# mborhi/CoMA-UNet

Measured on AMD Instinct MI355X. Metric: volumes/sec (train fwd+bwd) at 128^3 bf16, higher is better.
Workload: dtype bf16; 1 GPU; CoMA-UNet train step (fwd + RoiMSE/RnC loss + bwd + all-reduce + AdamW), 128^3 volumes, batch 2/GPU, 6-dim covariates (BASELINE configs[3]); global_batch=2, parallelism=dp1, launch=hipGraph replay of the whole step

## Files before the change

### coma_unet_amd/csrc/conv_mfma.hip

```cpp
#include "common.h"
#include "conv_tiles.h"
#include <type_traits>

template <typename T> struct elem;
template <> struct elem<bf16_t> { static constexpr int EPB = 8; };
template <> struct elem<float> { static constexpr int EPB = 4; };

__device__ __forceinline__ f32x16_t mma_piece(const uint4& a, const uint4& b, f32x16_t acc, bf16_t) {
  return __builtin_amdgcn_mfma_f32_32x32x16_bf16(*reinterpret_cast<const bf16x8_t*>(&a), *reinterpret_cast<const bf16x8_t*>(&b), acc, 0, 0, 0);
}
__device__ __forceinline__ f32x16_t mma_piece(const uint4& a, const uint4& b, f32x16_t acc, float) {
  acc = __builtin_amdgcn_mfma_f32_32x32x2f32(__uint_as_float(a.x), __uint_as_float(b.x), acc, 0, 0, 0);
  acc = __builtin_amdgcn_mfma_f32_32x32x2f32(__uint_as_float(a.y), __uint_as_float(b.y), acc, 0, 0, 0);
  acc = __builtin_amdgcn_mfma_f32_32x32x2f32(__uint_as_float(a.z), __uint_as_float(b.z), acc, 0, 0, 0);
  acc = __builtin_amdgcn_mfma_f32_32x32x2f32(__uint_as_float(a.w), __uint_as_float(b.w), acc, 0, 0, 0);
  return acc;
}

struct GatherP {
  const void* x; int ldx; long sbx; int Di, Hi, Wi, C;
  void* y; int ldy; long sby; int Do, Ho, Wo, N;
  const void* w; long wsb;
  const float* bias; int bsb;
  int k, stride, flip;
// ... 1072 lines not shown
        }
        const char* Wc = Wl + ((ph >> 1) & 1) * WB + w_frag;
        constexpr int NXR = LX == 5 ? 4 : 5;
        uint4 wg[2][3], xr[2][NXR];
        auto rdg = [&](int g, int bf) {
          const int kz = g / 3, kx = g % 3;
          const int toff = (kz * HY * HX + kx) * P;
#pragma unroll
          for (int r = 0; r < NXR; ++r) xr[bf][r] = *reinterpret_cast<const uint4*>(Hl + a_base + toff + r * HX * P);
#pragma unroll
          for (int ky = 0; ky < 3; ++ky) wg[bf][ky] = *reinterpret_cast<const uint4*>(Wc + (kz * 9 + ky * 3 + kx) * 1024);
        };
        rdg(0, 0);
#pragma unroll
        for (int g = 0; g < 9; ++g) {
          if (g + 1 < 9) rdg(g + 1, (g + 1) & 1);
#pragma unroll
          for (int ky = 0; ky < 3; ++ky)
#pragma unroll
            for (int i = 0; i < 2; ++i) acc[i] = mma_piece(wg[g & 1][ky], xr[g & 1][RY * i + ky], acc[i], bf16_t());
          __builtin_amdgcn_sched_group_barrier(0x008, 1, 0); __builtin_amdgcn_sched_group_barrier(0x100, 2, 0);
          __builtin_amdgcn_sched_group_barrier(0x008, 1, 0); __builtin_amdgcn_sched_group_barrier(0x100, 2, 0);
          __builtin_amdgcn_sched_group_barrier(0x008, 1, 0); __builtin_amdgcn_sched_group_barrier(0x100, 1, 0);
          __builtin_amdgcn_sched_group_barrier(0x008, 1, 0); __builtin_amdgcn_sched_group_barrier(0x100, 1, 0);
          __builtin_amdgcn_sched_group_barrier(0x008, 1, 0); __builtin_amdgcn_sched_group_barrier(0x100, 1, 0);
          __builtin_amdgcn_sched_group_barrier(0x008, 1, 0);
          __builtin_amdgcn_sched_barrier(0);
        }
      }
  };
  auto other_phase = [&](auto odd_c, int ph) __attribute__((always_inline)) {
      constexpr int odd = decltype(odd_c)::value;
#ifdef COMA_DUO_NO_STAGE
      if (cC.valid && cC.cc == nch - 1) {
#pragma unroll
        for (int i = 0; i < 2; ++i) asm volatile("" :: "v"(acc[i]));
      }
      cC = cB; advance(cB);
      return;
#endif
      store_halo(odd_c);
      const int ws = (ph >> 1) + 1;
      if (w_needed(ws)) store_w(ws);
      __builtin_amdgcn_s_waitcnt(0x0F70);
      if constexpr (odd == 0) {
#ifdef COMA_DUO_NO_EPI
      if (cC.valid && cC.cc == nch - 1) {
#pragma unroll
        for (int i = 0; i < 2; ++i) asm volatile("" :: "v"(acc[i]));
      }
#else
      if (cC.valid && cC.cc == nch - 1) {
        const int x0 = cC.tix * TX, y0 = cC.tiy * TY, z0 = cC.tiz * TZ;
        float4 bq[4];
#pragma unroll
        for (int g4 = 0; g4 < 4; ++g4) bq[g4] = *reinterpret_cast<const float4*>(bias_l + 8 * g4 + 4 * fh);
#pragma unroll
        for (int i = 0; i < 2; ++i) {
          const int j = wq * 2 + i;
          const int gz = z0 + (j >> 2), gy = y0 + (j & 3) * RY + (fr >> LX), gx = x0 + (fr & (TX - 1));
          const bool valid = gz < p.D && gy < p.H && gx < p.W;
          unsigned pk[4][2];
#pragma unroll
          for (int g4 = 0; g4 < 4; ++g4) {
            bf16_t o[4];
            const float bv[4] = {bq[g4].x, bq[g4].y, bq[g4].z, bq[g4].w};
#pragma unroll
            for (int q = 0; q < 4; ++q) {
              o[q] = static_cast<bf16_t>(acc[i][g4 * 4 + q] + bv[q]);
              if constexpr (STATS) {
                const float r = valid ? static_cast<float>(o[q]) : 0.f;
                st_s[g4][q] += r; st_q[g4][q] = fmaf(r, r, st_q[g4][q]);
              }
            }
            const uint2 u = *reinterpret_cast<const uint2*>(o);
            pk[g4][0] = u.x; pk[g4][1] = u.y;
          }
          bf16_t* vox = yb + ((long)(gz * p.H + gy) * p.W + gx) * p.ldy + n0 + 8 * fh;
#pragma unroll
          for (int gp = 0; gp < 2; ++gp) {
            const auto r0 = __builtin_amdgcn_permlane32_swap(pk[2 * gp][0], pk[2 * gp + 1][0], false, false);
            const auto r1 = __builtin_amdgcn_permlane32_swap(pk[2 * gp][1], pk[2 * gp + 1][1], false, false);
            if (valid) *reinterpret_cast<uint4*>(vox + 16 * gp) = make_uint4(r0[0], r1[0], r0[1], r1[1]);
          }
          __builtin_amdgcn_sched_barrier(0);
        }
      }
#endif
      }
      cC = cB; advance(cB);
      if constexpr (odd == 1) { load_halo(cA); advance2(cA); }
      if (w_needed(ws + 1)) load_w(ws + 1, true);
  };
  __builtin_amdgcn_s_waitcnt(0x0F70);
  if (grp == 0) {
#pragma unroll 1
    for (int ph = 0; ph < nphases; ph += 4) {
      matrix_phase(ph); duo_barrier(); other_phase(odd_t{}, ph + 1); duo_barrier();
      matrix_phase(ph + 2); duo_barrier(); other_phase(even_t{}, ph + 3); duo_barrier();
    }
  } else {
#pragma unroll 1
    for (int ph = 0; ph < nphases; ph += 4) {
      other_phase(even_t{}, ph); duo_barrier(); matrix_phase(ph + 1); duo_barrier();
      other_phase(odd_t{}, ph + 2); duo_barrier(); matrix_phase(ph + 3); duo_barrier();
    }
  }

  if constexpr (STATS) {
    if (p.stats) {
      asm volatile("s_waitcnt vmcnt(0)" ::: "memory");
      __syncthreads();
      float* red = reinterpret_cast<float*>(smem);
#pragma unroll
      for (int g4 = 0; g4 < 4; ++g4)
#pragma unroll
        for (int q = 0; q < 4; ++q) {
          float a = st_s[g4][q], c = st_q[g4][q];
#pragma unroll
          for (int o = 16; o > 0; o >>= 1) { a += __shfl_xor(a, o, 64); c += __shfl_xor(c, o, 64); }
          if (fr == 0) { red[(wid * 32 + 8 * g4 + 4 * fh + q) * 2] = a; red[(wid * 32 + 8 * g4 + 4 * fh + q) * 2 + 1] = c; }
        }
      __syncthreads();
      if (tid < 32 && n0 + tid < p.N) {
        double a = 0.0, c = 0.0;
        for (int w = 0; w < 8; ++w) { a += (double)red[(w * 32 + tid) * 2]; c += (double)red[(w * 32 + tid) * 2 + 1]; }
        const int g = p.stats_inst ? b : 0;
        stat_add(p.stats, p.stats_inst ? p.stats_inst : 1, p.N, g, n0 + tid, a, c);
      }
    }
  }
}

typedef __attribute__((ext_vector_type(4))) float f32x4_t;

struct Thin16P {
  const bf16_t* x; int ldx; long sbx; int D, H, W, C;
  bf16_t* y; int ldy; long sby; int N;
  const bf16_t* w; long wsb;
  const float* bias; int bsb;
  int flip;
  unsigned xbytes;
  int ntx, nty, ntz, ids_total, ids_per_block;
  int st8;
  double2* stats; int stats_inst;
};

template <int CP, int NB>
__global__ __launch_bounds__(256, 2) void conv_thin16_k(Thin16P p) {
  constexpr int TX = 32, TY = 4, TZ = 2, HX = TX + 2, HY = TY + 2, HZ = TZ + 2, HV = HX * HY * HZ;
  constexpr int TPM = 32 / CP, NM = (27 + TPM - 1) / TPM;
  constexpr int PCH = CP / 8;
  constexpr int P = CP * 2;
  constexpr int HP = HV * PCH, HIT = (HP + 255) / 256;
  extern __shared__ __attribute__((aligned(16))) char smem[];
  char* Hl = smem;
  const int tid = threadIdx.x, lane = tid & 63;
  const int wid = __builtin_amdgcn_readfirstlane(tid >> 6);
  const int b = blockIdx.z;
#ifdef COMA_STAMPS
  unsigned long long st_acc[8] = {0, 0, 0, 0, 0, 0, 0, 0};
  const unsigned long long st_begin = stamp_now();
  bool st_first = true;
#endif
  const int lv = lane & 15, lg = lane >> 4;
  const bf16_t* xb = p.x + (long)b * p.sbx;
  const bf16_t* wb = p.w + (long)b * p.wsb;
  bf16_t* yb = p.y + (long)b * p.sby;

  const int tsub = CP == 16 ? lg >> 1 : lg, cofs = CP == 16 ? 8 * (lg & 1) : 0;
  {
    const int total = 27 * p.N * p.C;
    unsigned short* Wl = reinterpret_cast<unsigned short*>(smem);
    const unsigned short* wg = reinterpret_cast<const unsigned short*>(wb);
    if ((total & 7) == 0 && (((uintptr_t)wg) & 15) == 0) {
      for (int i = tid; i < (total >> 3); i += 256) reinterpret_cast<uint4*>(Wl)[i] = reinterpret_cast<const uint4*>(wg)[i];
    } else {
      for (int i = tid; i < total; i += 256) Wl[i] = wg[i];
    }
  }
  __syncthreads();
  bf16x8_t wf[NM][NB];
#pragma unroll
  for (int m = 0; m < NM; ++m) {
    const int tap = m * TPM + tsub;
    const int wt = p.flip ? 26 - tap : tap;
#pragma unroll
    for (int nb = 0; nb < NB; ++nb) {
      const int n = nb * 16 + lv;
      unsigned short e[8];
#pragma unroll
      for (int j = 0; j < 8; ++j) {
        const int c = cofs + j;
        const bool ok = tap < 27 && n < p.N && c < p.C;
        const unsigned short v = reinterpret_cast<const unsigned short*>(smem)[ok ? (wt * p.N + n) * p.C + c : 0];
        e[j] = ok ? v : (unsigned short)0;
      }
      wf[m][nb] = (bf16x8_t){(short)e[0], (short)e[1], (short)e[2], (short)e[3], (short)e[4], (short)e[5], (short)e[6], (short)e[7]};
    }
  }
  const int gz = wid >> 1, gy0 = 2 * (wid & 1);
  int abase[NM];
#pragma unroll
  for (int m = 0; m < NM; ++m) {
    const int tap = m * TPM + tsub < 27 ? m * TPM + tsub : 0;
    const int kx = tap % 3, ky = (tap / 3) % 3, kz = tap / 9;
    abase[m] = (((gz + kz) * HY + gy0 + ky) * HX + lv + kx) * P + cofs * 2;
  }
  const __amdgpu_buffer_rsrc_t rs_x = __builtin_amdgcn_make_buffer_rsrc(const_cast<bf16_t*>(xb), 0, p.xbytes, 0x00020000);
  constexpr unsigned OOB = 0x7fff0000u;
  int h_z[HIT], h_y[HIT], h_x[HIT], h_lds[HIT];
  unsigned h_boff[HIT];
#pragma unroll
  for (int it = 0; it < HIT; ++it) {
    const int piece = tid + 256 * it;
    const int row = piece / PCH, ch = piece % PCH;
    const int hx = row % HX, hy = (row / HX) % HY, hz = row / (HX * HY);
    h_z[it] = piece < HP ? hz : (1 << 20); h_y[it] = hy; h_x[it] = hx;
#ifdef COMA_ABLATE_HALO
    if (hz < 1 || hz > TZ || hy < 1 || hy > TY || hx < 1 || hx > TX) h_z[it] = 1 << 20;
#endif
    h_boff[it] = (unsigned)((((hz * p.H + hy) * p.W + hx) * p.ldx + ch * 8) * 2);
    h_lds[it] = row * P + ch * 16;
  }
  const uint4 hmask = mask8(p.C - 8 * (tid % PCH));
  uint4 hreg[HIT];
  auto issue = [&](int it, int z0, int y0, int x0) __attribute__((always_inline)) {
    const bool ok = (unsigned)(z0 - 1 + h_z[it]) < (unsigned)p.D && (unsigned)(y0 - 1 + h_y[it]) < (unsigned)p.H &&
                    (unsigned)(x0 - 1 + h_x[it]) < (unsigned)p.W;
    const unsigned org_b = (unsigned)((((long)((z0 - 1) * p.H + (y0 - 1)) * p.W + (x0 - 1)) * p.ldx) * 2);
    const auto v = __builtin_amdgcn_raw_buffer_load_b128(rs_x, ok ? org_b + h_boff[it] : OOB, 0, 0);
    hreg[it] = make_uint4(v[0], v[1], v[2], v[3]);
  };
  auto store_halo = [&]() __attribute__((always_inline)) {
#pragma unroll
    for (int it = 0; it < HIT; ++it)
      if (tid + 256 * it < HP) {
        const uint4 m = hmask;
        uint4 v = hreg[it];
        v.x &= m.x; v.y &= m.y; v.z &= m.z; v.w &= m.w;
        *reinterpret_cast<uint4*>(Hl + h_lds[it]) = v;
      }
  };

  const int id_begin = xcd_remap(blockIdx.x, gridDim.x) * p.ids_per_block;
  int id_end = id_begin + p.ids_per_block;
  if (id_end > p.ids_total) id_end = p.ids_total;
  int id = id_begin, tix = 0, tiy = 0, tiz = 0;
  while (id < id_end && !tile_coords(id, p.ntx, p.nty, p.ntz, tix, tiy, tiz)) ++id;
  const bool do_stats = p.stats != nullptr;
  float st_s[NB][4], st_q[NB][4], bv[NB][4];
#pragma unroll
  for (int nb = 0; nb < NB; ++nb)
#pragma unroll
    for (int j = 0; j < 4; ++j) {
      const int n = nb * 16 + 4 * lg + j;
      st_s[nb][j] = 0.f; st_q[nb][j] = 0.f;
      bv[nb][j] = (p.bias && n < p.N) ? p.bias[b * p.bsb + n] : 0.f;
    }
  if (id < id_end) {
#pragma unroll
    for (int it = 0; it < HIT; ++it) issue(it, tiz * TZ, tiy * TY, tix * TX);
  }
  while (id < id_end) {
    const int x0 = tix * TX, y0 = tiy * TY, z0 = tiz * TZ;
    int nid = id + 1, ntix = 0, ntiy = 0, ntiz = 0;
    while (nid < id_end && !tile_coords(nid, p.ntx, p.nty, p.ntz, ntix, ntiy, ntiz)) ++nid;
    const bool has_next = nid < id_end;
    const __amdgpu_buffer_rsrc_t rs_n = __builtin_amdgcn_make_buffer_rsrc(const_cast<bf16_t*>(xb), 0, has_next ? p.xbytes : 0, 0x00020000);
    STAMP(t0);
#ifdef COMA_STAMPS
    if (st_first) { st_acc[0] += t0 - st_begin; st_first = false; }
#endif
    __syncthreads();
    STAMP(t1);
#ifdef COMA_STAMPS
    asm volatile("s_waitcnt vmcnt(0)" ::: "memory");
#endif
    STAMP(t2);
    store_halo();
    __syncthreads();
    STAMP(t3);
    f32x4_t acc[4][NB];
#pragma unroll
    for (int q = 0; q < 4; ++q)
#pragma unroll
      for (int nb = 0; nb < NB; ++nb) acc[q][nb] = (f32x4_t){0.f, 0.f, 0.f, 0.f};
    uint4 fr[3][4];
    auto ldfrag = [&](int m, int q) __attribute__((always_inline)) {
      return *reinterpret_cast<const uint4*>(Hl + abase[m] + ((q >> 1) * HX + (q & 1) * 16) * P);
    };
#pragma unroll
    for (int q = 0; q < 4; ++q) { fr[0][q] = ldfrag(0, q); fr[1][q] = ldfrag(1, q); }
#pragma unroll
    for (int m = 0; m < NM; ++m) {
      if (m + 2 < NM) {
#pragma unroll
        for (int q = 0; q < 4; ++q) fr[(m + 2) % 3][q] = ldfrag(m + 2, q);
      }
      if (m < HIT) {
        const int it = m;
        const bool ok = (unsigned)(ntiz * TZ - 1 + h_z[it]) < (unsigned)p.D && (unsigned)(ntiy * TY - 1 + h_y[it]) < (unsigned)p.H &&
                        (unsigned)(ntix * TX - 1 + h_x[it]) < (unsigned)p.W;
        const unsigned org_b = (unsigned)((((long)((ntiz * TZ - 1) * p.H + (ntiy * TY - 1)) * p.W + (ntix * TX - 1)) * p.ldx) * 2);
        const auto v = __builtin_amdgcn_raw_buffer_load_b128(rs_n, ok ? org_b + h_boff[it] : OOB, 0, 0);
        hreg[it] = make_uint4(v[0], v[1], v[2], v[3]);
      }
      __builtin_amdgcn_sched_barrier(0);
#ifdef COMA_ABLATE_MFMA
      if (m > 0) continue;
#endif
#pragma unroll
      for (int q = 0; q < 4; ++q) {
        const uint4 f = fr[m % 3][q];
#pragma unroll
        for (int nb = 0; nb < NB; ++nb)
          acc[q][nb] = __builtin_amdgcn_mfma_f32_16x16x32_bf16(wf[m][nb], *reinterpret_cast<const bf16x8_t*>(&f), acc[q][nb], 0, 0, 0);
      }
      __builtin_amdgcn_sched_barrier(0);
    }
    static_assert(HIT <= NM, "one staging piece per MFMA step");
    STAMP(t4);
#pragma unroll
    for (int q = 0; q < 4; ++q) {
      const int vz = z0 + gz, vy = y0 + gy0 + (q >> 1), vx = x0 + (q & 1) * 16 + lv;
      const bool valid = vz < p.D && vy < p.H && vx < p.W;
      bf16_t* vox = yb + ((long)(vz * p.H + vy) * p.W + vx) * p.ldy;
#pragma unroll
      for (int nb = 0; nb < NB; ++nb) {
        const int n = nb * 16 + 4 * lg;
        if (n >= p.N) continue;
        bf16_t o[4];
#pragma unroll
        for (int j = 0; j < 4; ++j) {
          o[j] = static_cast<bf16_t>(acc[q][nb][j] + bv[nb][j]);
          if (do_stats) { const float r = valid ? static_cast<float>(o[j]) : 0.f; st_s[nb][j] += r; st_q[nb][j] = fmaf(r, r, st_q[nb][j]); }
        }
#ifdef COMA_ABLATE_STORE
        if (valid && acc[q][nb][0] == 123.456f) {
#else
        if (valid) {
#endif
          if (p.st8 && n + 3 < p.N) *reinterpret_cast<uint2*>(vox + n) = *reinterpret_cast<const uint2*>(o);
          else {
#pragma unroll
            for (int j = 0; j < 4; ++j) if (n + j < p.N) vox[n + j] = o[j];
          }
        }
      }
    }
    id = nid; tix = ntix; tiy = ntiy; tiz = ntiz;
    STAMP(t5);
    STAMP_ADD(1, t0, t1); STAMP_ADD(2, t1, t2); STAMP_ADD(3, t2, t3); STAMP_ADD(4, t3, t4); STAMP_ADD(5, t4, t5);
  }
#ifdef COMA_STAMPS
  {
    const unsigned long long st_end = stamp_now();
    if (lane == 0) {
      for (int k = 0; k < 7; ++k) atomicAdd(&g_stamps[k], st_acc[k]);
      atomicAdd(&g_stamps[7], st_end - st_begin);
      atomicAdd(&g_stamps[8], 1ull);
    }
  }
#endif
  if (p.stats) {
    __syncthreads();
    float* red = reinterpret_cast<float*>(smem);
#pragma unroll
    for (int nb = 0; nb < NB; ++nb)
#pragma unroll
      for (int j = 0; j < 4; ++j) {
        float a = st_s[nb][j], c = st_q[nb][j];
#pragma unroll
        for (int o = 8; o > 0; o >>= 1) { a += __shfl_xor(a, o, 64); c += __shfl_xor(c, o, 64); }
        if (lv == 0) { red[(wid * 32 + nb * 16 + 4 * lg + j) * 2] = a; red[(wid * 32 + nb * 16 + 4 * lg + j) * 2 + 1] = c; }
      }
    __syncthreads();
    if (tid < NB * 16 && tid < p.N) {
      double a = 0.0, c = 0.0;
      for (int w = 0; w < 4; ++w) { a += (double)red[(w * 32 + tid) * 2]; c += (double)red[(w * 32 + tid) * 2 + 1]; }
      const int g = p.stats_inst ? b : 0;
      stat_add(p.stats, p.stats_inst ? p.stats_inst : 1, p.N, g, tid, a, c);
    }
  }
}

struct Thin16FP {
  const float* x; int ldx; long sbx; int D, H, W, C;
  float* y; int ldy; long sby; int N;
  const float* w; long wsb;
  const float* bias; int bsb;
  int flip;
  unsigned xbytes;
  int ntx, nty, ntz, ids_total, ids_per_block;
  int st16;
  double2* stats; int stats_inst;
};

template <int CP, int NB>
__global__ __launch_bounds__(256, 2) void conv_thin16f_k(Thin16FP p) {
  constexpr int TX = 32, TY = 4, TZ = 2, HX = TX + 2, HY = TY + 2, HZ = TZ + 2, HV = HX * HY * HZ;
  constexpr int CQ = CP / 4;
  constexpr int P = CP * 4;
  constexpr int PCH = CP / 4;
  constexpr int HP = HV * PCH, HIT = (HP + 255) / 256;
  constexpr int WROW = NB * 16;
  extern __shared__ __attribute__((aligned(16))) char smem[];
  char* Hl = smem;
  float* Wl = reinterpret_cast<float*>(smem + HV * P);
  const int tid = threadIdx.x, lane = tid & 63;
  const int wid = __builtin_amdgcn_readfirstlane(tid >> 6);
  const int b = blockIdx.z;
  const int lv = lane & 15, lg = lane >> 4;
  const float* xb = p.x + (long)b * p.sbx;
  const float* wb = p.w + (long)b * p.wsb;
  float* yb = p.y + (long)b * p.sby;

  for (int i = tid; i < 27 * WROW * CP; i += 256) {
    const int c = i % CP, n = (i / CP) % WROW, t = i / (CP * WROW);
    const int wt = p.flip ? 26 - t : t;
    const bool ok = n < p.N && c < p.C;
    const float v = wb[ok ? ((long)wt * p.N + n) * p.C + c : 0];
    Wl[i] = ok ? v : 0.f;
  }
  const int gz = wid >> 1, gy0 = 2 * (wid & 1);
  const int xbase = ((gz * HY + gy0) * HX + lv) * P + lg * CQ * 4;
  const int wbase = (lv * CP + lg * CQ) * 4;
  const __amdgpu_buffer_rsrc_t rs_x = __builtin_amdgcn_make_buffer_rsrc(const_cast<float*>(xb), 0, p.xbytes, 0x00020000);
  constexpr unsigned OOB = 0x7fff0000u;
  int h_z[HIT], h_y[HIT], h_x[HIT];
  unsigned h_boff[HIT];
#pragma unroll
  for (int it = 0; it < HIT; ++it) {
    const int piece = tid + 256 * it;
    const int row = piece / PCH, ch = piece % PCH;
    const int hx = row % HX, hy = (row / HX) % HY, hz = row / (HX * HY);
    h_z[it] = piece < HP ? hz : (1 << 20); h_y[it] = hy; h_x[it] = hx;
    h_boff[it] = (unsigned)((((hz * p.H + hy) * p.W + hx) * p.ldx + ch * 4) * 4);
  }
  const int nval = p.C - 4 * (tid % PCH);
  const uint4 hmask = make_uint4(nval > 0 ? ~0u : 0u, nval > 1 ? ~0u : 0u, nval > 2 ? ~0u : 0u, nval > 3 ? ~0u : 0u);
  uint4 hreg[HIT];
  auto store_halo = [&]() __attribute__((always_inline)) {
#pragma unroll
    for (int it = 0; it < HIT; ++it)
      if (tid + 256 * it < HP) {
        uint4 v = hreg[it];
        v.x &= hmask.x; v.y &= hmask.y; v.z &= hmask.z; v.w &= hmask.w;
        *reinterpret_cast<uint4*>(Hl + (tid + 256 * it) * 16) = v;
      }
  };

  const int id_begin = xcd_remap(blockIdx.x, gridDim.x) * p.ids_per_block;
  int id_end = id_begin + p.ids_per_block;
  if (id_end > p.ids_total) id_end = p.ids_total;
  int id = id_begin, tix = 0, tiy = 0, tiz = 0;
  while (id < id_end && !tile_coords(id, p.ntx, p.nty, p.ntz, tix, tiy, tiz)) ++id;
  const bool do_stats = p.stats != nullptr;
  float st_s[NB][4], st_q[NB][4], bv[NB][4];
#pragma unroll
  for (int nb = 0; nb < NB; ++nb)
#pragma unroll
    for (int j = 0; j < 4; ++j) {
      const int n = nb * 16 + 4 * lg + j;
      st_s[nb][j] = 0.f; st_q[nb][j] = 0.f;
      bv[nb][j] = (p.bias && n < p.N) ? p.bias[b * p.bsb + n] : 0.f;
    }
  if (id < id_end) {
#pragma unroll
    for (int it = 0; it < HIT; ++it) {
      const int z0 = tiz * TZ, y0 = tiy * TY, x0 = tix * TX;
      const bool ok = (unsigned)(z0 - 1 + h_z[it]) < (unsigned)p.D && (unsigned)(y0 - 1 + h_y[it]) < (unsigned)p.H &&
                      (unsigned)(x0 - 1 + h_x[it]) < (unsigned)p.W;
      const unsigned org_b = (unsigned)((((long)((z0 - 1) * p.H + (y0 - 1)) * p.W + (x0 - 1)) * p.ldx) * 4);
      const auto v = __builtin_amdgcn_raw_buffer_load_b128(rs_x, ok ? org_b + h_boff[it] : OOB, 0, 0);
      hreg[it] = make_uint4(v[0], v[1], v[2], v[3]);
    }
  }
  while (id < id_end) {
    const int x0 = tix * TX, y0 = tiy * TY, z0 = tiz * TZ;
    int nid = id + 1, ntix = 0, ntiy = 0, ntiz = 0;
    while (nid < id_end && !tile_coords(nid, p.ntx, p.nty, p.ntz, ntix, ntiy, ntiz)) ++nid;
    const bool has_next = nid < id_end;
    const __amdgpu_buffer_rsrc_t rs_n = __builtin_amdgcn_make_buffer_rsrc(const_cast<float*>(xb), 0, has_next ? p.xbytes : 0, 0x00020000);
    __syncthreads();
    store_halo();
    __syncthreads();
    f32x4_t acc[4][NB];
#pragma unroll
    for (int q = 0; q < 4; ++q)
#pragma unroll
      for (int nb = 0; nb < NB; ++nb) acc[q][nb] = (f32x4_t){0.f, 0.f, 0.f, 0.f};
    float xf[2][4][CQ], wfr[2][NB][CQ];
    auto rd = [&](int t, int bf) __attribute__((always_inline)) {
      const int toff = (((t / 9) * HY + (t / 3) % 3) * HX + t % 3) * P;
#pragma unroll
      for (int q = 0; q < 4; ++q) {
        const char* src = Hl + xbase + toff + ((q >> 1) * HX + (q & 1) * 16) * P;
        if constexpr (CQ == 4) { const float4 v = *reinterpret_cast<const float4*>(src); xf[bf][q][0] = v.x; xf[bf][q][1] = v.y; xf[bf][q][2] = v.z; xf[bf][q][3] = v.w; }
        else if constexpr (CQ == 2) { const float2 v = *reinterpret_cast<const float2*>(src); xf[bf][q][0] = v.x; xf[bf][q][1] = v.y; }
        else xf[bf][q][0] = *reinterpret_cast<const float*>(src);
      }
#pragma unroll
      for (int nb = 0; nb < NB; ++nb) {
        const char* src = reinterpret_cast<const char*>(Wl) + wbase + (t * WROW + nb * 16) * CP * 4;
        if constexpr (CQ == 4) { const float4 v = *reinterpret_cast<const float4*>(src); wfr[bf][nb][0] = v.x; wfr[bf][nb][1] = v.y; wfr[bf][nb][2] = v.z; wfr[bf][nb][3] = v.w; }
// ... 622 lines not shown
    (void)hipFuncSetAttribute((const void*)conv_mfma_tconv_k<float, true>, hipFuncAttributeMaxDynamicSharedMemorySize, 160 * 1024);
    attr = true;
  }
  const size_t lds = (size_t)(33 * 5 * 3 + 14 * 32) * 80;
  coma_set_kernel_tag("conv_mfma_tconv_k<%s, %d>", sizeof(T) == 2 ? "__bf16" : "float", q.stats ? 1 : 0);
  const dim3 grid((unsigned)gx, (unsigned)nblk_n, (unsigned)x->B);
  if (q.stats) hipLaunchKernelGGL((conv_mfma_tconv_k<T, true>), grid, dim3(256), lds, s, q);
  else hipLaunchKernelGGL((conv_mfma_tconv_k<T, false>), grid, dim3(256), lds, s, q);
  COMA_LAUNCH_CHECK();
  return 0;
}

bool conv_mfma_supported(const coma_conv_desc* d, const coma_tensor* x, const coma_tensor* y) {
  if (x->dtype != COMA_BF16 || y->dtype != COMA_BF16) return false;
  if ((long)t_vox(x) * x->ld >= (1L << 31) || (long)t_vox(y) * y->ld >= (1L << 31)) return false;
  if (halo_ok(d, x, y)) return true;
  if (pw_ok(d, x, y)) return true;
  if (x->C % 32 || y->C % 32) return false;
  if (x->ld % 8 || y->ld % 8 || x->sb % 8 || y->sb % 8) return false;
  if (x->data && !aligned16(x->data)) return false;
  if ((long)t_vox(x) * x->ld >= (1L << 31) || (long)t_vox(y) * y->ld >= (1L << 31)) return false;
  if (d->form == 1 && d->stride == 2 && d->ksize != 3) return false;
  return true;
}

static bool f32_halo_ok(const coma_conv_desc* d, const coma_tensor* x, const coma_tensor* y) {
  if (x->W < 16 && x->C % 32 == 0 && y->C % 32 == 0) return false;
  return d->ksize == 3 && d->stride == 1 && x->W >= 8 && (long)x->H * x->W >= 32 && x->C % 16 == 0 && y->C >= 16 &&
         x->ld % 4 == 0 && x->sb % 4 == 0 && (!x->data || aligned16(x->data)) && (unsigned long long)t_vox(x) * x->ld * 4 < 0x7fff0000ull;
}
bool conv_f32mfma_supported(const coma_conv_desc* d, const coma_tensor* x, const coma_tensor* y) {
  if (x->dtype != COMA_F32 || y->dtype != COMA_F32) return false;
  if ((long)t_vox(x) * x->ld >= (1L << 31) || (long)t_vox(y) * y->ld >= (1L << 31)) return false;
  if (thin16f_ok(d, x, y)) return true;
  if (f32_halo_ok(d, x, y)) return true;
  if (x->C % 16 || y->C % 32) return false;
  if (x->ld % 4 || y->ld % 4 || x->sb % 4 || y->sb % 4) return false;
  if (x->data && !aligned16(x->data)) return false;
  if (d->form == 1 && d->stride == 2 && d->ksize != 3) return false;
  return true;
}

static int gather_ksplit(long blocks, int nsteps, bool f32) {
  if (f32) {
    if (blocks >= 192 || nsteps < 8) return 1;
    long ks = 256 / blocks;
    if (ks > 8) ks = 8;
    if (ks > nsteps / 4) ks = nsteps / 4;
    return ks < 2 ? 1 : (int)ks;
  }
  if (blocks >= 384 || nsteps < 16) return 1;
  long ks = 512 / blocks;
  if (ks > 8) ks = 8;
  if (ks > nsteps / 4) ks = nsteps / 4;
  return ks < 2 ? 1 : (int)ks;
}

template <int BN, typename T>
static int launch_gather(const GatherP& p0, int mode, int B, hipStream_t s, void* ws, size_t ws_bytes, int ws_zeroed,
                         double2* stats, int stats_inst, int* stats_chunks) {
  GatherP p = p0;
  constexpr int BM = (BN == 128) ? 128 : 256;
  constexpr int LCK = elem<T>::EPB == 8 ? 5 : 4;
  const long Mtot = (long)p.Mz * p.My * p.Mx;
  const size_t lds = (size_t)2 * (BM + BN) * 64 + BM * 4;
  const unsigned gx = (unsigned)((Mtot + BM - 1) / BM), gy = (unsigned)(p.N / BN) * (mode == 1 ? 8 : 1);
  const long Vout = (long)p.Do * p.Ho * p.Wo;
  const int ntaps_max = mode == 1 ? 8 : p.k * p.k * p.k;
  p.ksplit = gather_ksplit((long)gx * gy * B, (mode == 1 ? 1 : ntaps_max) * (p.C >> LCK), LCK == 4);
  p.part = nullptr; p.part_sb = 0;
  if (p.ksplit > 1 && ws && ws_bytes >= sizeof(float) * (size_t)B * Vout * p.N) {
    p.part = (float*)ws; p.part_sb = Vout * p.N;
    if (!ws_zeroed && hipMemsetAsync(ws, 0, sizeof(float) * (size_t)B * Vout * p.N, s) != hipSuccess) { coma_set_error("conv split-K memset failed"); return 2; }
  } else p.ksplit = 1;
  p.stats = nullptr; p.stats_inst = stats_inst;
  if (stats && p.ksplit == 1 && !p.accum) { p.stats = stats; *stats_chunks = 1; }
  dim3 grid(gx, gy * p.ksplit, (unsigned)B);
  coma_set_kernel_tag("conv_mfma_gather_k<%d, %d, %s>", BN, mode, LCK == 4 ? "float" : "__bf16");
  if (mode == 0) hipLaunchKernelGGL((conv_mfma_gather_k<BN, 0, T>), grid, dim3(256), lds, s, p);
  else hipLaunchKernelGGL((conv_mfma_gather_k<BN, 1, T>), grid, dim3(256), lds, s, p);
  COMA_LAUNCH_CHECK();
  if (p.ksplit > 1) {
    long nb = (Vout * p.N + 255) / 256;
    if (nb > 1024) nb = 1024;
    hipLaunchKernelGGL(gather_finalize_k<T>, dim3((unsigned)nb, (unsigned)B), dim3(256), 0, s, (const float*)p.part, p.part_sb, (T*)p.y, p.ldy,
                       p.sby, p.N, Vout, p.bias, p.bsb, p.accum);
    COMA_LAUNCH_CHECK();
  }
  return 0;
}

template <int CK, int LX, int VEC, typename T>
static int launch_halo(const HaloP& p0, int B, hipStream_t s) {
  HaloP p = p0;
  constexpr int TX = 1 << LX, RY = 32 / TX, TY = 4 * RY, TZ = 2;
  constexpr int HV = (TX + 2) * (TY + 2) * (TZ + 2);
  p.ntx = (p.W + TX - 1) / TX; p.nty = (p.H + TY - 1) / TY; p.ntz = (p.D + TZ - 1) / TZ;
  const size_t lds = (size_t)(HV + 9 * 32) * CK * sizeof(T);
  static bool attr = false;
  if (!attr) { (void)hipFuncSetAttribute((const void*)conv_mfma_halo_k<CK, LX, VEC, T>, hipFuncAttributeMaxDynamicSharedMemorySize, 96 * 1024); attr = true; }
  dim3 grid((unsigned)(p.ntx * p.nty * ((p.ntz + 7) / 8) * 8), (unsigned)((p.N + 31) / 32), (unsigned)B);
  coma_set_kernel_tag("conv_mfma_halo_k<%d, %d, %d, %s>", CK, LX, VEC, sizeof(T) == 4 ? "float" : "__bf16");
  hipLaunchKernelGGL((conv_mfma_halo_k<CK, LX, VEC, T>), grid, dim3(256), lds, s, p);
  COMA_LAUNCH_CHECK();
  return 0;
}

static bool aligned16(const void* p);
static size_t duo_frag_bytes(const coma_conv_desc* d, const coma_tensor* x, const coma_tensor* y) {
  static const bool on = getenv("COMA_DUO_C32_ONLY") == nullptr && getenv("COMA_NO_DUO") == nullptr;
  if (!on || x->dtype != COMA_BF16 || d->ksize != 3 || d->stride != 1 || x->W < 16) return 0;
  if (x->C < 64 || x->C % 16 || y->C % 32) return 0;
  return (size_t)(d->per_sample_w ? x->B : 1) * 27 * y->C * x->C * 2;
}

template <typename T>
static int conv_mfma_halo(const coma_conv_desc* d, const coma_tensor* x, const void* wk, const float* bias,
                          const coma_tensor* y, hipStream_t s, double2* stats = nullptr, int stats_inst = 0,
                          int* stats_chunks = nullptr, void* ws = nullptr, size_t ws_bytes = 0) {
  constexpr int EPB = elem<T>::EPB;
  constexpr bool F32 = EPB == 4;
  HaloP p;
  p.x = x->data; p.ldx = (int)x->ld; p.sbx = x->sb; p.D = x->D; p.H = x->H; p.W = x->W; p.C = x->C;
  p.y = y->data; p.ldy = (int)y->ld; p.sby = y->sb; p.N = y->C;
  p.w = wk; p.wsb = d->per_sample_w ? 27L * y->C * x->C : 0;
  p.bias = bias; p.bsb = d->per_sample_w ? y->C : 0;
  p.flip = d->form == 1;
  p.vecx = x->ld % EPB == 0 && x->sb % EPB == 0 && aligned16(x->data);
  p.vecw = x->C % EPB == 0 && aligned16(wk);
  const bool thin = !F32 && x->C <= 16;
  const int lx = x->W >= 32 ? 5 : (x->W >= 16 ? 4 : 3);
  const bool vec = p.vecx && p.vecw && x->C % (4 * EPB) == 0 && (unsigned long long)t_vox(x) * x->ld * sizeof(T) < 0x7fff0000ull;
  if (F32) COMA_CHECK(vec, "conv_mfma(fp32): operands must allow 16-byte channel pieces (C %% 16 == 0, aligned)");
  if constexpr (!F32) {
    static const bool thin16_on = []{ const char* e = getenv("COMA_THIN16"); return !(e && e[0] == '0'); }();
    const unsigned long long xb_ = (unsigned long long)t_vox(x) * x->ld * sizeof(T);
    if (thin16_on && thin && lx == 5 && y->C <= (x->C > 8 ? 16 : 32) && p.vecx && xb_ < 0x7fff0000ull) {
      Thin16P q;
      q.x = (const bf16_t*)p.x; q.ldx = p.ldx; q.sbx = p.sbx; q.D = p.D; q.H = p.H; q.W = p.W; q.C = p.C;
      q.y = (bf16_t*)p.y; q.ldy = p.ldy; q.sby = p.sby; q.N = p.N; q.w = (const bf16_t*)p.w; q.wsb = p.wsb; q.bias = p.bias; q.bsb = p.bsb;
      q.flip = p.flip; q.xbytes = (unsigned)xb_;
      q.st8 = y->ld % 4 == 0 && y->sb % 4 == 0 && (((uintptr_t)y->data) & 7) == 0;
      q.ntx = (q.W + 31) / 32; q.nty = (q.H + 3) / 4; q.ntz = (q.D + 1) / 2;
      q.ids_total = q.ntx * q.nty * ((q.ntz + 7) / 8) * 8;
      int gx = 1024 / x->B;
      if (gx < 1) gx = 1;
      if (gx > q.ids_total) gx = q.ids_total;
      q.ids_per_block = (q.ids_total + gx - 1) / gx;
      gx = (q.ids_total + q.ids_per_block - 1) / q.ids_per_block;
      q.stats = nullptr; q.stats_inst = stats_inst;
      if (stats) { q.stats = stats; *stats_chunks = 1; }
      dim3 grid((unsigned)gx, 1, (unsigned)x->B);
      const bool c16 = q.C > 8, n32 = q.N > 16;
      size_t lds = (size_t)34 * 6 * 4 * (c16 ? 32 : 16);
      if (lds < (size_t)27 * q.N * q.C * 2) lds = (size_t)27 * q.N * q.C * 2;
      coma_set_kernel_tag("conv_thin16_k<%d, %d>", c16 ? 16 : 8, n32 ? 2 : 1);
      if (c16) hipLaunchKernelGGL((conv_thin16_k<16, 1>), grid, dim3(256), lds, s, q);
      else     { if (n32) hipLaunchKernelGGL((conv_thin16_k<8, 2>), grid, dim3(256), lds, s, q);  else hipLaunchKernelGGL((conv_thin16_k<8, 1>), grid, dim3(256), lds, s, q); }
      COMA_LAUNCH_CHECK();
      return 0;
    }
  }
  if ((lx == 5 && (thin || vec)) || (lx == 4 && !F32 && !thin && vec)) {
    Halo2P q;
    q.x = p.x; q.ldx = p.ldx; q.sbx = p.sbx; q.D = p.D; q.H = p.H; q.W = p.W; q.C = p.C;
    q.y = p.y; q.ldy = p.ldy; q.sby = p.sby; q.N = p.N; q.w = p.w; q.wsb = p.wsb; q.bias = p.bias; q.bsb = p.bsb;
    q.flip = p.flip; q.vecx = p.vecx; q.vecw = p.vecw;
    {
      const unsigned long long xb_ = (unsigned long long)t_vox(x) * x->ld * sizeof(T), wb_ = 27ull * y->C * x->C * sizeof(T);
      q.xbytes = (unsigned)(xb_ < 0x7fff0000ull ? xb_ : 0x7fff0000ull);
      q.wbytes = (unsigned)(wb_ < 0x7fff0000ull ? wb_ : 0x7fff0000ull);
    }
    q.stats = nullptr; q.stats_inst = stats_inst;
    q.st8 = y->ld % 4 == 0 && y->sb % 4 == 0 && (((uintptr_t)y->data) & 7) == 0;
    q.st16 = y->ld % EPB == 0 && y->sb % EPB == 0 && (((uintptr_t)y->data) & 15) == 0;
    const int txv = lx == 5 ? 32 : 16, tyv = lx == 5 ? 4 : 8;
    q.ntx = (q.W + txv - 1) / txv; q.nty = (q.H + tyv - 1) / tyv; q.ntz = (q.D + 1) / 2;
    q.ids_total = q.ntx * q.nty * ((q.ntz + 7) / 8) * 8;
    const int nblk_n = (q.N + 31) / 32;
    int gx = (thin ? 1024 : 512) / (nblk_n * x->B);
    if (F32) gx = 256 / (nblk_n * x->B);
    if (gx < 1) gx = 1;
    if (gx > q.ids_total) gx = q.ids_total;
    q.ids_per_block = (q.ids_total + gx - 1) / gx;
    gx = (q.ids_total + q.ids_per_block - 1) / q.ids_per_block;
    dim3 grid((unsigned)gx, (unsigned)nblk_n, (unsigned)x->B);
    if (stats) { q.stats = stats; *stats_chunks = 1; }
    if constexpr (!F32) {
      static const bool no_duo = getenv("COMA_NO_DUO") != nullptr, duo_all = getenv("COMA_DUO_C32_ONLY") == nullptr;
      q.wfrag = nullptr; q.wfrag_sb = 0;
      const size_t frag_bytes = duo_frag_bytes(d, x, y);
      const bool wide_ok = duo_all && q.C > 32 && frag_bytes > 0 && ws && ws_bytes >= frag_bytes && aligned16(ws);
      if (!no_duo && !thin && vec && (q.C == 32 || wide_ok) && q.N % 32 == 0 && q.st16 &&
          q.D <= 510 && q.H <= 510 && q.W <= 510) {
        if (q.C > 32) {
          const long pieces = (long)(frag_bytes / 16);
          hipLaunchKernelGGL(duo_relayout_k, dim3((unsigned)((pieces + 255) / 256)), dim3(256), 0, s, (const uint4*)wk, (uint4*)ws, q.N, q.C / 8, pieces);
          COMA_LAUNCH_CHECK();
          q.wfrag = ws; q.wfrag_sb = d->per_sample_w ? 27L * q.N * q.C : 0;
        }
        int g2 = 256 / (nblk_n * x->B);
        if (g2 < 1) g2 = 1;
        if (g2 > q.ids_total) g2 = q.ids_total;
        q.ids_per_block = (q.ids_total + g2 - 1) / g2;
        g2 = (q.ids_total + q.ids_per_block - 1) / q.ids_per_block;
        const dim3 grid2((unsigned)g2, (unsigned)nblk_n, (unsigned)x->B);
        if (stats) { q.stats = stats; *stats_chunks = 1; }
        const size_t lds2 = (size_t)2 * 34 * 6 * 4 * 48 + (size_t)2 * 27 * 64 * 16 + 128;
        static bool attr2 = false;
        if (!attr2) {
          (void)hipFuncSetAttribute((const void*)conv_mfma_duo_k<0, 5>, hipFuncAttributeMaxDynamicSharedMemorySize, 160 * 1024);
          (void)hipFuncSetAttribute((const void*)conv_mfma_duo_k<1, 5>, hipFuncAttributeMaxDynamicSharedMemorySize, 160 * 1024);
          (void)hipFuncSetAttribute((const void*)conv_mfma_duo_k<0, 4>, hipFuncAttributeMaxDynamicSharedMemorySize, 160 * 1024);
          (void)hipFuncSetAttribute((const void*)conv_mfma_duo_k<1, 4>, hipFuncAttributeMaxDynamicSharedMemorySize, 160 * 1024);
          attr2 = true;
        }
        if (lx == 5) {
          coma_set_kernel_tag("conv_mfma_duo_k<%d, 5>", stats ? 1 : 0);
          if (stats) hipLaunchKernelGGL((conv_mfma_duo_k<1, 5>), grid2, dim3(512), lds2, s, q);
          else hipLaunchKernelGGL((conv_mfma_duo_k<0, 5>), grid2, dim3(512), lds2, s, q);
        } else {
          coma_set_kernel_tag("conv_mfma_duo_k<%d, 4>", stats ? 1 : 0);
          if (stats) hipLaunchKernelGGL((conv_mfma_duo_k<1, 4>), grid2, dim3(512), lds2, s, q);
          else hipLaunchKernelGGL((conv_mfma_duo_k<0, 4>), grid2, dim3(512), lds2, s, q);
        }
        COMA_LAUNCH_CHECK();
        return 0;
      }
    }
    if (lx == 5) {
    constexpr int HV2 = 34 * 6 * 4;
    const bool resident = thin || (!F32 && q.C == 32);
    const size_t lds = thin ? (size_t)(HV2 + 27 * 32) * 48 : (size_t)HV2 * 80 + (size_t)27 * 32 * 80;
    static bool attr = false;
    if (!attr) {
      if constexpr (F32) {
        (void)hipFuncSetAttribute((const void*)conv_mfma_halo2_k<2, 16, 1, 1, float>, hipFuncAttributeMaxDynamicSharedMemorySize, 160 * 1024);
      } else {
        (void)hipFuncSetAttribute((const void*)conv_mfma_halo2_k<1, 32, 1, 1>, hipFuncAttributeMaxDynamicSharedMemorySize, 160 * 1024);
        (void)hipFuncSetAttribute((const void*)conv_mfma_halo2_k<2, 32, 1, 1>, hipFuncAttributeMaxDynamicSharedMemorySize, 160 * 1024);
        (void)hipFuncSetAttribute((const void*)conv_mfma_halo2_k<1, 16, 0, 2>, hipFuncAttributeMaxDynamicSharedMemorySize, 80 * 1024);
      }
      attr = true;
    }
    coma_set_kernel_tag(F32 ? "conv_mfma_halo2_k<2, 16, 1, 1, float>" : thin ? "conv_mfma_halo2_k<1, 16, 0, 2, __bf16>"
                        : resident ? "conv_mfma_halo2_k<1, 32, 1, 1, __bf16>" : "conv_mfma_halo2_k<2, 32, 1, 1, __bf16>");
    if constexpr (F32) {
      hipLaunchKernelGGL((conv_mfma_halo2_k<2, 16, 1, 1, float>), grid, dim3(256), lds, s, q);
    } else {
      if (thin) hipLaunchKernelGGL((conv_mfma_halo2_k<1, 16, 0, 2>), grid, dim3(256), lds, s, q);
      else if (resident) hipLaunchKernelGGL((conv_mfma_halo2_k<1, 32, 1, 1>), grid, dim3(256), lds, s, q);
      else hipLaunchKernelGGL((conv_mfma_halo2_k<2, 32, 1, 1>), grid, dim3(256), lds, s, q);
    }
    COMA_LAUNCH_CHECK();
    return 0;
    }
    if (stats_chunks) *stats_chunks = 0;
  }
  if constexpr (F32) {
    if (lx == 5) return launch_halo<16, 5, 1, float>(p, x->B, s);
    if (lx == 4) return launch_halo<16, 4, 1, float>(p, x->B, s);
    return launch_halo<16, 3, 1, float>(p, x->B, s);
  } else {
    if (thin) {
      if (lx == 5) return launch_halo<16, 5, 0, bf16_t>(p, x->B, s);
      if (lx == 4) return launch_halo<16, 4, 0, bf16_t>(p, x->B, s);
      return launch_halo<16, 3, 0, bf16_t>(p, x->B, s);
    }
    if (vec) {
      if (lx == 5) return launch_halo<32, 5, 1, bf16_t>(p, x->B, s);
      if (lx == 4) return launch_halo<32, 4, 1, bf16_t>(p, x->B, s);
      return launch_halo<32, 3, 1, bf16_t>(p, x->B, s);
    }
    if (lx == 5) return launch_halo<32, 5, 0, bf16_t>(p, x->B, s);
    if (lx == 4) return launch_halo<32, 4, 0, bf16_t>(p, x->B, s);
    return launch_halo<32, 3, 0, bf16_t>(p, x->B, s);
  }
}

bool conv_mfma_accumulate_ok(const coma_conv_desc* d, const coma_tensor* x, const coma_tensor* y) {
  if (x->dtype == COMA_F32) return conv_f32mfma_supported(d, x, y) && !thin16f_ok(d, x, y) && !f32_halo_ok(d, x, y);
  return conv_mfma_supported(d, x, y) && !halo_ok(d, x, y);
}

static int gather_ksplit(long blocks, int nsteps, bool f32);
size_t conv_mfma_fwd_ws_bytes(const coma_conv_desc* d, const coma_tensor* x, const coma_tensor* y) {
  if (x->dtype == COMA_F32) { if (thin16f_ok(d, x, y) || f32_halo_ok(d, x, y)) return 0; }
  else if (halo_ok(d, x, y)) return duo_frag_bytes(d, x, y);
  else if (pw_ok(d, x, y)) return 0;
  if (tconv_ok(d, x, y)) return 0;
  const size_t bytes = sizeof(float) * (size_t)y->B * t_vox(y) * y->C;
  if (bytes > ((size_t)64 << 20)) return 0;
  const bool f32 = x->dtype == COMA_F32;
  const int BN = y->C % 128 == 0 ? 128 : y->C % 64 == 0 ? 64 : 32, BM = BN == 128 ? 128 : 256, LCK = f32 ? 4 : 5;
  const int mode = d->form == 1 && d->stride == 2;
  const long Mtot = mode ? (long)((y->D + 1) / 2) * ((y->H + 1) / 2) * ((y->W + 1) / 2) : (long)t_vox(y);
  const long gx = (Mtot + BM - 1) / BM, gy = (long)(y->C / BN) * (mode ? 8 : 1);
  const int taps = d->ksize * d->ksize * d->ksize;
  return gather_ksplit(gx * gy * y->B, (mode ? 1 : taps) * (x->C >> LCK), f32) > 1 ? bytes : 0;
}

int conv_mfma_fwd(const coma_conv_desc* d, const coma_tensor* x, const void* wk, const float* bias,
                  const coma_tensor* y, hipStream_t s, double2* stats, int stats_inst, int* stats_chunks, void* ws,
                  size_t ws_bytes, int ws_zeroed, int accum) {
  const bool f32 = x->dtype == COMA_F32;
  COMA_CHECK(!accum || conv_mfma_accumulate_ok(d, x, y), "conv_mfma: this problem's kernel family cannot accumulate into y");
  if (f32 && thin16f_ok(d, x, y)) return conv_thin16f(d, x, wk, bias, y, s, stats, stats_inst, stats_chunks);
// ... 1634 lines not shown
```

Before: 117.2 volumes/s.

## Reuse z-halo planes across consecutive tiles via three-slot LDS ring in thin16 conv

The thin-channel 3x3x3 conv kernel now splits each tile's 4-plane halo into two 2-plane units held in a 3-slot LDS ring. When the next tile is the z-successor, only one new plane pair is loaded and the overlapping pair is reused. Refills are issued after the MFMA loop and stored into the ring. This is meant to cut global halo traffic and staging stores roughly in half for z-contiguous tile runs. In exchange, LDS grows from 4 to 6 planes, which may reduce occupancy, and the slot and continuity bookkeeping is more complex.

```diff
diff --git a/coma_unet_amd/csrc/conv_mfma.hip b/coma_unet_amd/csrc/conv_mfma.hip
--- a/coma_unet_amd/csrc/conv_mfma.hip
+++ b/coma_unet_amd/csrc/conv_mfma.hip
@@ -1248,7 +1248,9 @@
   constexpr int TPM = 32 / CP, NM = (27 + TPM - 1) / TPM;
   constexpr int PCH = CP / 8;
   constexpr int P = CP * 2;
-  constexpr int HP = HV * PCH, HIT = (HP + 255) / 256;
+  constexpr int UP = 2 * HY * HX * PCH, UIT = (UP + 255) / 256;
+  constexpr int UB = 2 * HY * HX * P, RB = 3 * UB;
+  static_assert(HZ == 4, "a tile reads two plane pairs");
   extern __shared__ __attribute__((aligned(16))) char smem[];
   char* Hl = smem;
   const int tid = threadIdx.x, lane = tid & 63;
@@ -1304,38 +1306,40 @@
     abase[m] = (((gz + kz) * HY + gy0 + ky) * HX + lv + kx) * P + cofs * 2;
   }
   const __amdgpu_buffer_rsrc_t rs_x = __builtin_amdgcn_make_buffer_rsrc(const_cast<bf16_t*>(xb), 0, p.xbytes, 0x00020000);
+  const __amdgpu_buffer_rsrc_t rs_0 = __builtin_amdgcn_make_buffer_rsrc(const_cast<bf16_t*>(xb), 0, 0, 0x00020000);
   constexpr unsigned OOB = 0x7fff0000u;
-  int h_z[HIT], h_y[HIT], h_x[HIT], h_lds[HIT];
-  unsigned h_boff[HIT];
-#pragma unroll
-  for (int it = 0; it < HIT; ++it) {
+  int h_z[UIT], h_y[UIT], h_x[UIT], h_lds[UIT];
+  unsigned h_boff[UIT];
+#pragma unroll
+  for (int it = 0; it < UIT; ++it) {
     const int piece = tid + 256 * it;
     const int row = piece / PCH, ch = piece % PCH;
     const int hx = row % HX, hy = (row / HX) % HY, hz = row / (HX * HY);
-    h_z[it] = piece < HP ? hz : (1 << 20); h_y[it] = hy; h_x[it] = hx;
-#ifdef COMA_ABLATE_HALO
-    if (hz < 1 || hz > TZ || hy < 1 || hy > TY || hx < 1 || hx > TX) h_z[it] = 1 << 20;
-#endif
+    h_z[it] = piece < UP ? hz : (1 << 20); h_y[it] = hy - 1; h_x[it] = hx - 1;
     h_boff[it] = (unsigned)((((hz * p.H + hy) * p.W + hx) * p.ldx + ch * 8) * 2);
     h_lds[it] = row * P + ch * 16;
   }
   const uint4 hmask = mask8(p.C - 8 * (tid % PCH));
-  uint4 hreg[HIT];
-  auto issue = [&](int it, int z0, int y0, int x0) __attribute__((always_inline)) {
-    const bool ok = (unsigned)(z0 - 1 + h_z[it]) < (unsigned)p.D && (unsigned)(y0 - 1 + h_y[it]) < (unsigned)p.H &&
-                    (unsigned)(x0 - 1 + h_x[it]) < (unsigned)p.W;
-    const unsigned org_b = (unsigned)((((long)((z0 - 1) * p.H + (y0 - 1)) * p.W + (x0 - 1)) * p.ldx) * 2);
-    const auto v = __builtin_amdgcn_raw_buffer_load_b128(rs_x, ok ? org_b + h_boff[it] : OOB, 0, 0);
-    hreg[it] = make_uint4(v[0], v[1], v[2], v[3]);
-  };
-  auto store_halo = [&]() __attribute__((always_inline)) {
-#pragma unroll
-    for (int it = 0; it < HIT; ++it)
-      if (tid + 256 * it < HP) {
+  uint4 hreg[UIT];
+  auto issue_unit = [&](int zp, int y0, int x0, const __amdgpu_buffer_rsrc_t& rs) __attribute__((always_inline)) {
+    const unsigned org_b = (unsigned)((((long)(zp * p.H + (y0 - 1)) * p.W + (x0 - 1)) * p.ldx) * 2);
+#pragma unroll
+    for (int it = 0; it < UIT; ++it) {
+      const bool ok = (unsigned)(zp + h_z[it]) < (unsigned)p.D && (unsigned)(y0 + h_y[it]) < (unsigned)p.H &&
+                      (unsigned)(x0 + h_x[it]) < (unsigned)p.W;
+      const auto v = __builtin_amdgcn_raw_buffer_load_b128(rs, ok ? org_b + h_boff[it] : OOB, 0, 0);
+      hreg[it] = make_uint4(v[0], v[1], v[2], v[3]);
+    }
+  };
+  auto store_unit = [&](int slot) __attribute__((always_inline)) {
+    char* dst = Hl + slot * UB;
+#pragma unroll
+    for (int it = 0; it < UIT; ++it)
+      if (tid + 256 * it < UP) {
         const uint4 m = hmask;
         uint4 v = hreg[it];
         v.x &= m.x; v.y &= m.y; v.z &= m.z; v.w &= m.w;
-        *reinterpret_cast<uint4*>(Hl + h_lds[it]) = v;
+        *reinterpret_cast<uint4*>(dst + h_lds[it]) = v;
       }
   };
 
@@ -1344,6 +1348,8 @@
   if (id_end > p.ids_total) id_end = p.ids_total;
   int id = id_begin, tix = 0, tiy = 0, tiz = 0;
   while (id < id_end && !tile_coords(id, p.ntx, p.nty, p.ntz, tix, tiy, tiz)) ++id;
+  int nid = id + 1, ntix = 0, ntiy = 0, ntiz = 0;
+  while (nid < id_end && !tile_coords(nid, p.ntx, p.nty, p.ntz, ntix, ntiy, ntiz)) ++nid;
   const bool do_stats = p.stats != nullptr;
   float st_s[NB][4], st_q[NB][4], bv[NB][4];
 #pragma unroll
@@ -1354,54 +1360,53 @@
       st_s[nb][j] = 0.f; st_q[nb][j] = 0.f;
       bv[nb][j] = (p.bias && n < p.N) ? p.bias[b * p.bsb + n] : 0.f;
     }
+  __syncthreads();
+  int cs = 1;
+  bool fresh = true;
   if (id < id_end) {
-#pragma unroll
-    for (int it = 0; it < HIT; ++it) issue(it, tiz * TZ, tiy * TY, tix * TX);
+    issue_unit(tiz * TZ - 1, tiy * TY, tix * TX, rs_x);
+    store_unit(0);
+    issue_unit(tiz * TZ + 1, tiy * TY, tix * TX, rs_x);
   }
   while (id < id_end) {
     const int x0 = tix * TX, y0 = tiy * TY, z0 = tiz * TZ;
-    int nid = id + 1, ntix = 0, ntiy = 0, ntiz = 0;
-    while (nid < id_end && !tile_coords(nid, p.ntx, p.nty, p.ntz, ntix, ntiy, ntiz)) ++nid;
-    const bool has_next = nid < id_end;
-    const __amdgpu_buffer_rsrc_t rs_n = __builtin_amdgcn_make_buffer_rsrc(const_cast<bf16_t*>(xb), 0, has_next ? p.xbytes : 0, 0x00020000);
+    const bool has1 = nid < id_end;
+    const bool cont1 = has1 && ntix == tix && ntiy == tiy && ntiz == tiz + 1;
+    int mid = nid + 1, mtix = 0, mtiy = 0, mtiz = 0;
+    while (mid < id_end && !tile_coords(mid, p.ntx, p.nty, p.ntz, mtix, mtiy, mtiz)) ++mid;
+    const bool has2 = mid < id_end;
+    const bool cont2 = has2 && mtix == ntix && mtiy == ntiy && mtiz == ntiz + 1;
+    const int zp1 = cont1 ? ntiz * TZ + 1 : ntiz * TZ - 1;
     STAMP(t0);
 #ifdef COMA_STAMPS
     if (st_first) { st_acc[0] += t0 - st_begin; st_first = false; }
 #endif
+    if (fresh) {
+      __syncthreads();
+      store_unit(cs);
+      issue_unit(zp1, ntiy * TY, ntix * TX, has1 ? rs_x : rs_0);
+      __builtin_amdgcn_sched_barrier(0);
+    }
     __syncthreads();
     STAMP(t1);
-#ifdef COMA_STAMPS
-    asm volatile("s_waitcnt vmcnt(0)" ::: "memory");
-#endif
-    STAMP(t2);
-    store_halo();
-    __syncthreads();
-    STAMP(t3);
     f32x4_t acc[4][NB];
 #pragma unroll
     for (int q = 0; q < 4; ++q)
 #pragma unroll
       for (int nb = 0; nb < NB; ++nb) acc[q][nb] = (f32x4_t){0.f, 0.f, 0.f, 0.f};
+    const int sbase = (cs == 0 ? 2 : cs - 1) * UB;
     uint4 fr[3][4];
-    auto ldfrag = [&](int m, int q) __attribute__((always_inline)) {
-      return *reinterpret_cast<const uint4*>(Hl + abase[m] + ((q >> 1) * HX + (q & 1) * 16) * P);
+    auto ldfrag4 = [&](int m, uint4 (&dst)[4]) __attribute__((always_inline)) {
+      int a = abase[m] + sbase;
+      a = a >= RB ? a - RB : a;
+#pragma unroll
+      for (int q = 0; q < 4; ++q) dst[q] = *reinterpret_cast<const uint4*>(Hl + a + ((q >> 1) * HX + (q & 1) * 16) * P);
     };
-#pragma unroll
-    for (int q = 0; q < 4; ++q) { fr[0][q] = ldfrag(0, q); fr[1][q] = ldfrag(1, q); }
+    ldfrag4(0, fr[0]);
+    if (NM > 1) ldfrag4(1, fr[1]);
 #pragma unroll
     for (int m = 0; m < NM; ++m) {
-      if (m + 2 < NM) {
-#pragma unroll
-        for (int q = 0; q < 4; ++q) fr[(m + 2) % 3][q] = ldfrag(m + 2, q);
-      }
-      if (m < HIT) {
-        const int it = m;
-        const bool ok = (unsigned)(ntiz * TZ - 1 + h_z[it]) < (unsigned)p.D && (unsigned)(ntiy * TY - 1 + h_y[it]) < (unsigned)p.H &&
-                        (unsigned)(ntix * TX - 1 + h_x[it]) < (unsigned)p.W;
-        const unsigned org_b = (unsigned)((((long)((ntiz * TZ - 1) * p.H + (ntiy * TY - 1)) * p.W + (ntix * TX - 1)) * p.ldx) * 2);
-        const auto v = __builtin_amdgcn_raw_buffer_load_b128(rs_n, ok ? org_b + h_boff[it] : OOB, 0, 0);
-        hreg[it] = make_uint4(v[0], v[1], v[2], v[3]);
-      }
+      if (m + 2 < NM) ldfrag4(m + 2, fr[(m + 2) % 3]);
       __builtin_amdgcn_sched_barrier(0);
 #ifdef COMA_ABLATE_MFMA
       if (m > 0) continue;
@@ -1415,7 +1420,18 @@
       }
       __builtin_amdgcn_sched_barrier(0);
     }
-    static_assert(HIT <= NM, "one staging piece per MFMA step");
+    STAMP(t2);
+#ifdef COMA_STAMPS
+    asm volatile("s_waitcnt vmcnt(0)" ::: "memory");
+#endif
+    STAMP(t3);
+    store_unit(cs == 2 ? 0 : cs + 1);
+    {
+      const bool up1 = has1 && !cont1;
+      const int zpn = up1 ? ntiz * TZ + 1 : (cont2 ? mtiz * TZ + 1 : mtiz * TZ - 1);
+      issue_unit(zpn, (up1 ? ntiy : mtiy) * TY, (up1 ? ntix : mtix) * TX, (up1 || has2) ? rs_x : rs_0);
+    }
+    __builtin_amdgcn_sched_barrier(0);
     STAMP(t4);
 #pragma unroll
     for (int q = 0; q < 4; ++q) {
@@ -1445,9 +1461,12 @@
         }
       }
     }
+    cs = cont1 ? (cs == 2 ? 0 : cs + 1) : (cs == 0 ? 2 : cs - 1);
+    fresh = !cont1;
     id = nid; tix = ntix; tiy = ntiy; tiz = ntiz;
+    nid = mid; ntix = mtix; ntiy = mtiy; ntiz = mtiz;
     STAMP(t5);
-    STAMP_ADD(1, t0, t1); STAMP_ADD(2, t1, t2); STAMP_ADD(3, t2, t3); STAMP_ADD(4, t3, t4); STAMP_ADD(5, t4, t5);
+    STAMP_ADD(1, t0, t1); STAMP_ADD(4, t1, t2); STAMP_ADD(2, t2, t3); STAMP_ADD(3, t3, t4); STAMP_ADD(5, t4, t5);
   }
 #ifdef COMA_STAMPS
   {
@@ -2376,7 +2395,7 @@
       if (stats) { q.stats = stats; *stats_chunks = 1; }
       dim3 grid((unsigned)gx, 1, (unsigned)x->B);
       const bool c16 = q.C > 8, n32 = q.N > 16;
-      size_t lds = (size_t)34 * 6 * 4 * (c16 ? 32 : 16);
+      size_t lds = (size_t)34 * 6 * 6 * (c16 ? 32 : 16);
       if (lds < (size_t)27 * q.N * q.C * 2) lds = (size_t)27 * q.N * q.C * 2;
       coma_set_kernel_tag("conv_thin16_k<%d, %d>", c16 ? 16 : 8, n32 ? 2 : 1);
       if (c16) hipLaunchKernelGGL((conv_thin16_k<16, 1>), grid, dim3(256), lds, s, q);
```

Measured after the change: 117.0 volumes/s. No clear change (-0.2%).
